# j-min/HiREST

Measured on AMD Instinct MI355X. Metric: encoded frames/sec (EVA-CLIP-g/14 224^2), higher is better.
Workload: dtype bf16

## Files before the change

### hirest_amd/_lib.py

```python
from __future__ import annotations

import ctypes as C
import os

HERE = os.path.dirname(os.path.abspath(__file__))
LIB_PATH = os.path.join(HERE, "lib", "libhirest_hip.so")
if os.environ.get("HIREST_LIB_VARIANT"):
    LIB_PATH = os.path.join(HERE, "lib", f"libhirest_hip.{os.environ['HIREST_LIB_VARIANT']}.so")

(EPI_BIAS_BF16, EPI_BIAS_GELU_BF16, EPI_BIAS_QGELU_BF16, EPI_BIAS_RESID_F32, EPI_BIAS_F32, EPI_PATCH_POS_F32,
 EPI_BIAS_RESID_LNSTATS_F32, EPI_LNFOLD_BF16, EPI_LNFOLD_GELU_BF16, EPI_BIAS_GELU_SPLIT2, EPI_BIAS_RESID2_LNSTATS) = range(11)

TOWER_NO_LNFOLD = 1
TOWER_NO_PRUNE = 2
TOWER_F32_RESIDUAL = 4
GEMM_REVERSE = 1
GEMM_X3 = 2
GEMM_X3_T128 = 4
ABI_VERSION = 4

ERRORS = {-1: "HIREST_E_BADARG", -2: "HIREST_E_SHAPE (unsupported shape)", -3: "HIREST_E_WORKSPACE (workspace too small)"}


class GemmArgs(C.Structure):
    _fields_ = [("struct_size", C.c_uint64),
                ("A", C.c_void_p), ("lda", C.c_int64), ("W", C.c_void_p), ("ldw", C.c_int64),
                ("bias", C.c_void_p), ("out", C.c_void_p), ("ldo", C.c_int64),
                ("M", C.c_int32), ("N", C.c_int32), ("K", C.c_int32), ("epilogue", C.c_int32),
                ("pos", C.c_void_p), ("patches_per_frame", C.c_int32), ("aux0", C.c_void_p), ("aux1", C.c_void_p), ("flags", C.c_int32)]

    @classmethod
    def make(cls, *fields):
        return cls(C.sizeof(cls), *fields)


F32_ENTRY = {"gemm": 0, "ws": 1, "layouts": 2, "ln": 3, "ln_colmax": 4, "rows_colmax": 5}


class GemmF32Query(C.Structure):
    _fields_ = [("struct_size", C.c_uint32)] + \
               [(n, C.c_int32) for n in ("entry", "M", "N", "K", "has_resid", "has_periodic", "has_ids", "has_ln_out", "has_workspace",
                                         "a_kmajor", "w_kmajor", "select_kernel", "ring_mode", "rows_ln_mode", "cus")]

    @classmethod
    def make(cls, entry, M, N, K, **fields):
        q = cls(C.sizeof(cls), F32_ENTRY[entry], M, N, K, select_kernel=-1, ring_mode=-1, rows_ln_mode=-1)
        for k, v in fields.items():
            setattr(q, k, int(v))
        return q


class BlockWeights(C.Structure):
    _fields_ = [(n, C.c_void_p) for n in ("ln1_g", "ln1_b", "qkv_w", "qkv_b", "proj_w", "proj_b",
                                          "ln2_g", "ln2_b", "fc1_w", "fc1_b", "fc2_w", "fc2_b",
                                          "qkv_wf", "qkv_bf", "qkv_s", "fc1_wf", "fc1_bf", "fc1_s")]


class VisionTower(C.Structure):
    _fields_ = [(n, C.c_int32) for n in ("image_size", "patch", "width", "heads", "head_dim", "mlp_dim",
                                         "layers", "embed_dim", "kpad", "act")] + \
               [("ln_eps", C.c_float)] + \
               [("patch_w", C.c_void_p), ("patch_b", C.c_void_p), ("cls", C.c_void_p), ("pos", C.c_void_p),
                ("blocks", C.POINTER(BlockWeights)),
                ("norm_g", C.c_void_p), ("norm_b", C.c_void_p), ("head_w", C.c_void_p), ("head_b", C.c_void_p),
                ("image_mean", C.c_void_p), ("image_std", C.c_void_p),
                ("ln_pre_g", C.c_void_p), ("ln_pre_b", C.c_void_p), ("out_all_tokens", C.c_int32)]


class TextTower(C.Structure):
    _fields_ = [(n, C.c_int32) for n in ("context", "vocab", "width", "heads", "layers", "embed_dim", "act")] + \
               [("ln_eps", C.c_float)] + \
# ... 495 lines not shown
```

### hirest_amd/csrc/gemm.hip

```cpp
#include <cstdio>
#include <atomic>
#include "gemm_shared.h"

namespace {


constexpr int BM = 128, BN = 128, BK = 64;
constexpr int STAGE_BYTES = (BM + BN) * BK * 2;

template <int EPI>
__device__ __forceinline__ void epilogue_store(const GemmP& p, int m, int n, f32x4 v) {
    if (p.bias) {
        f32x4 b = *reinterpret_cast<const f32x4*>(p.bias + n);
        v += b;
    }
    if constexpr (EPI == HIREST_EPI_BIAS_BF16 || EPI == HIREST_EPI_BIAS_GELU_BF16 || EPI == HIREST_EPI_BIAS_QGELU_BF16) {
        if constexpr (EPI == HIREST_EPI_BIAS_GELU_BF16) {
#pragma unroll
            for (int i = 0; i < 4; ++i) v[i] = gelu_erf(v[i]);
        }
        if constexpr (EPI == HIREST_EPI_BIAS_QGELU_BF16) {
#pragma unroll
            for (int i = 0; i < 4; ++i) v[i] = quick_gelu(v[i]);
        }
// ... 927 lines not shown
            if constexpr (epi_is_lnfold(EPI)) {
                int r0 = M0 + wr * 128 + 2 * lane;
                const int last = (p.M - 1) & ~1;
                r0 = r0 < last ? r0 : last;
                glds16(reinterpret_cast<const float*>(p.aux0) + 2 * (int64_t)r0, stg + P_STG);
            }
#pragma unroll
            for (int i = 0; i < 8; ++i)
#pragma unroll
                for (int jn = 0; jn < NI; ++jn) acc[i][jn] = f32x4{0.f, 0.f, 0.f, 0.f};
            load_frags(smem + (g & 1) * Q_STEP, 0, f0);
            for (int t = 0; t < nst; ++t, ++g) {
                const char* cur = smem + (g & 1) * Q_STEP;
                const char* nxt = smem + ((g + 1) & 1) * Q_STEP;
                __builtin_amdgcn_sched_barrier(0);
                if (!(dbg & 256)) load_frags(cur, 1, f1);
                mfma_half(f0);
#pragma unroll
                for (int i = 0; i < NR; ++i) {
                    __builtin_amdgcn_sched_group_barrier(0x008, 2, 0);
                    __builtin_amdgcn_sched_group_barrier(0x100, 1, 0);
                }
                __builtin_amdgcn_sched_barrier(0);
                if (!(dbg & 64)) HX_WAIT_VM(0);
                HX_WAIT_LGKM0();
                __builtin_amdgcn_s_barrier();
                __builtin_amdgcn_sched_barrier(0);
                stage();
                load_frags(nxt, 0, f0);
                mfma_half(f1);
                __builtin_amdgcn_sched_group_barrier(0x020, 2 * PPW, 0);
#pragma unroll
                for (int i = 0; i < NR; ++i) {
                    __builtin_amdgcn_sched_group_barrier(0x008, 1, 0);
                    __builtin_amdgcn_sched_group_barrier(0x100, 1, 0);
                }
                __builtin_amdgcn_sched_barrier(0);
                advance();
            }
            epilogue_p<EPI, NI, epi_is_lnfold(EPI), 8, RD, false, DBG>(p, acc, stg, M0 + wr * 128, N0 + wc * WN, lane);
        } else {
            for (int t = 0; t < nst; ++t, ++g) {
                HX_WAIT_VM(0);
                __builtin_amdgcn_s_barrier();
                stage();
                advance();
            }
        }
    }
    HX_WAIT_VM(0);
}


template <int EPI, int RD, bool X3, int PH2 = 0, bool DBG = false>
__device__ __forceinline__ void pp256_body(const GemmP& p) {
    constexpr int NI = 4;
    const int sched = DBG ? p.sched : 0, stagger = DBG ? p.stagger : 0;
    extern __shared__ __attribute__((aligned(16))) char smem[];
    const int tid = threadIdx.x, lane = tid & 63;
    const int wave = __builtin_amdgcn_readfirstlane(tid >> 6);
    const int grp = wave >> 2;
    const int wr = grp, wc = wave & 3;

    const int bid = blockIdx.x;
    const int xcd = bid & 7, slot = bid >> 3, nslot = gridDim.x >> 3;
    int p_lo, np;
    xcd_panels<DBG>(p, xcd, p_lo, np);
    if (np <= 0) return;
    const bool panel_major = p.nbn <= 8;
    const int nunit = np * p.nbn;
    if (slot >= nunit) return;
    const bool team_walk = DBG && (sched & 4) && panel_major && p.nbn <= nslot && nunit >= nslot;
    const int teams = team_walk ? nslot / p.nbn : 0, tslots = teams * p.nbn, solo = nslot - tslots;
    const int np_solo = team_walk && solo ? (np * solo + nslot / 2) / nslot : 0, np_team = np - np_solo;
    int count;
    if (!team_walk) count = (nunit - slot + nslot - 1) / nslot;
    else if (slot < tslots) { const int tm = slot / p.nbn; count = tm < np_team ? (np_team - tm + teams - 1) / teams : 0; }
    else { const int sl_ = slot - tslots; count = sl_ < np_solo ? ((np_solo - sl_ + solo - 1) / solo) * p.nbn : 0; }
    if (count <= 0) return;
    if (stagger) {
        const int who = stagger == 1 ? (slot & 3) : stagger == 2 ? (xcd & 3) : ((slot + xcd) & 7);
        const int units = who * (stagger == 3 ? (p.K / Q_BK + 15) / 16 : (p.K / Q_BK + 7) / 8);
        for (int i = 0; i < units; ++i) __builtin_amdgcn_s_sleep(127);
    }
    auto team_origin = [&](int i, int& M0, int& N0) {
        if (p.rev) i = count - 1 - i;
        int panel, col;
        if (slot < tslots) { panel = slot / p.nbn + i * teams; col = slot % p.nbn; }
        else { panel = np_team + (slot - tslots) + (i / p.nbn) * solo; col = i % p.nbn; }
        M0 = (p_lo + panel) * T_BM; N0 = col * T_BN;
    };
    auto tile_origin = [&](int j, int& M0, int& N0) {
        if (team_walk) { team_origin((j - slot) / nslot, M0, N0); return; }
        if (p.rev) j = nunit - 1 - j;
        if (panel_major) {
            const int mt_i = j / p.nbn;
            M0 = (p_lo + mt_i) * T_BM; N0 = (j - mt_i * p.nbn) * T_BN;
            return;
        }
        const int g_ = j / (GROUP_M * p.nbn);
        const int r = j - g_ * GROUP_M * p.nbn;
        int gcount = np - g_ * GROUP_M; gcount = gcount > GROUP_M ? GROUP_M : gcount;
        const int nt_i = r / gcount, mt_i = p_lo + g_ * GROUP_M + (r - nt_i * gcount);
        M0 = mt_i * T_BM; N0 = nt_i * T_BN;
    };

    const int nst = p.K / Q_BK;
    uint32_t a_off[2][2], w_off[2][2];
    int a_lds[2][2], w_lds[2][2];
    const char* a_base; const char* w_base;
#pragma unroll
    for (int hsel = 0; hsel < 2; ++hsel)
#pragma unroll
        for (int q = 0; q < 2; ++q) {
            const int j = 2 * wave + q;
            a_lds[hsel][q] = ((j >> 3) * 128 + hsel * 64 + (j & 7) * 8) * 128;
            w_lds[hsel][q] = Q_WOFF + ((j >> 2) * 64 + hsel * 32 + (j & 3) * 8) * 128;
        }
    auto set_sources = [&](int M0, int N0) {
#pragma unroll
        for (int hsel = 0; hsel < 2; ++hsel)
#pragma unroll
            for (int q = 0; q < 2; ++q) {
                const int ra0 = (a_lds[hsel][q] >> 7) + (lane >> 3);
                const int rw0 = ((w_lds[hsel][q] - Q_WOFF) >> 7) + (lane >> 3);
                const int ca = (lane & 7) ^ ((ra0 >> 1) & 7), cw = (lane & 7) ^ ((rw0 >> 1) & 7);
                int ra = p.M - 1 - M0; ra = ra0 < ra ? ra0 : ra;
                int rn = p.N - 1 - N0; rn = rw0 < rn ? rw0 : rn;
                a_off[hsel][q] = (uint32_t)(ra * (int)p.lda + ca * 8) * 2u;
                w_off[hsel][q] = (uint32_t)(rn * (int)p.ldw + cw * 8) * 2u;
            }
        const int Ma = (DBG && (sched & 8)) ? (p_lo + ((M0 / T_BM - p_lo) & 3)) * T_BM : M0;
// ... 28 lines not shown
            dma_j += nslot;
            if (dma_j < slot + count * nslot) { int m0, n0; tile_origin(dma_j, m0, n0); set_sources(m0, n0); dma_k = 0; }
            else { dma_live = false; dma_k = nst - 1; }
        }
    };

    const int frow = lane & 15, fsw = (frow >> 1) & 7, kg = lane >> 4;
    const int a_frag = (wr * 128 + frow) * (Q_BK * 2);
    const int w_frag = Q_WOFF + (wc * 64 + frow) * (Q_BK * 2);
    int koff[2];
#pragma unroll
    for (int h = 0; h < 2; ++h) koff[h] = ((4 * h + kg) ^ fsw) << 4;
    struct FA { bf16x8 v[4][2]; };
    struct FW { bf16x8 v[2][2]; };
    FA Af;
    FW W0, W1;
    auto read_a = [&](const char* buf, int a) {
#pragma unroll
        for (int m = 0; m < 4; ++m)
#pragma unroll
            for (int h = 0; h < 2; ++h) Af.v[m][h] = *reinterpret_cast<const bf16x8*>(buf + a_frag + (a * 64 + m * 16) * 128 + koff[h]);
    };
    auto read_w = [&](const char* buf, int b, FW& f) {
#pragma unroll
        for (int n = 0; n < 2; ++n)
#pragma unroll
            for (int h = 0; h < 2; ++h) f.v[n][h] = *reinterpret_cast<const bf16x8*>(buf + w_frag + (b * 32 + n * 16) * 128 + koff[h]);
    };
    f32x4 acc[8][NI];
    auto mfma_q = [&](int a, int b, FW& fw) {
        __builtin_amdgcn_s_setprio(1);
        if constexpr (X3) {
#pragma unroll
            for (int g3 = 0; g3 < 3; ++g3)
#pragma unroll
                for (int m = 0; m < 4; ++m)
#pragma unroll
                    for (int n = 0; n < 2; ++n)
                        acc[a * 4 + m][b * 2 + n] = __builtin_amdgcn_mfma_f32_16x16x32_bf16(fw.v[n][g3 == 1 ? 1 : 0], Af.v[m][g3 == 0 ? 1 : 0],
                                                                                             acc[a * 4 + m][b * 2 + n], 0, 0, 0);
        } else {
#pragma unroll
            for (int h = 0; h < 2; ++h)
#pragma unroll
                for (int m = 0; m < 4; ++m)
#pragma unroll
                    for (int n = 0; n < 2; ++n)
                        acc[a * 4 + m][b * 2 + n] = __builtin_amdgcn_mfma_f32_16x16x32_bf16(fw.v[n][h], Af.v[m][h], acc[a * 4 + m][b * 2 + n], 0, 0, 0);
        }
        __builtin_amdgcn_s_setprio(0);
    };
    auto bar = [&]() { __builtin_amdgcn_s_barrier(); };

    {
        int m0, n0;
        tile_origin(slot, m0, n0);
        set_sources(m0, n0);
    }
    for (int i = 0; i < 2; ++i) { issue_a0(); issue_w(0); issue_w(1); advance(); issue_a1_pending(); }
    bool a1_valid = false;
    HX_WAIT_VM(0);
    bar();
    if (grp == 1) bar();

    char* stg = smem + 2 * Q_STEP + wave * p_stg_bytes(EPI);
    int g = 0;
    for (int j = slot; j < slot + count * nslot; j += nslot) {
        int M0, N0;
        tile_origin(j, M0, N0);
        const bool active = (N0 + wc * 64 < p.N) && (M0 + wr * 128 < p.M);
        if (active) {
            if constexpr (epi_is_lnfold(EPI)) {
                int r0 = M0 + wr * 128 + 2 * lane;
                const int last = (p.M - 1) & ~1;
                r0 = r0 < last ? r0 : last;
                glds16(reinterpret_cast<const float*>(p.aux0) + 2 * (int64_t)r0, stg + P_STG);
                int c = N0 + wc * 64 + 4 * (lane & 15);
                c = c < p.N - 4 ? c : p.N - 4;
                const float* src = ((lane & 16) || !p.bias) ? reinterpret_cast<const float*>(p.aux1) : p.bias;
                glds16(src + c, stg + P_BCS);
            }
#pragma unroll
            for (int i = 0; i < 8; ++i)
#pragma unroll
                for (int jn = 0; jn < NI; ++jn) acc[i][jn] = f32x4{0.f, 0.f, 0.f, 0.f};
        }
        if (active && PH2) {
            for (int t = 0; t < nst; ++t, ++g) {
                const char* cur = smem + (g & 1) * Q_STEP;
                HX_WAIT_VM(6);
                __builtin_amdgcn_sched_barrier(0);
                read_a(cur, 0); read_w(cur, 0, W0); read_w(cur, 1, W1);
                if (a1_valid) issue_a1_pending();
                HX_WAIT_LGKM0();
                bar();
                mfma_q(0, 0, W0);
                mfma_q(0, 1, W1);
                bar();
                HX_WAIT_VM(2);
                __builtin_amdgcn_sched_barrier(0);
                read_a(cur, 1);
                issue_a0(); issue_w(0); issue_w(1);
                advance();
                a1_valid = true;
                HX_WAIT_LGKM0();
                bar();
// ... 18 lines not shown
                const char* cur = smem + (g & 1) * Q_STEP;
                HX_WAIT_VM(8);
                __builtin_amdgcn_sched_barrier(0);
                read_a(cur, 0); read_w(cur, 0, W0);
                if (a1_valid) issue_a1_pending();
                bar();
                HX_WAIT_LGKM0();
                mfma_q(0, 0, W0);
                bar();
                HX_WAIT_VM(8);
                __builtin_amdgcn_sched_barrier(0);
                read_w(cur, 1, W1);
                bar();
                HX_WAIT_LGKM0();
                mfma_q(0, 1, W1);
                bar();
                __builtin_amdgcn_sched_barrier(0);
                read_a(cur, 1);
                issue_a0(); issue_w(0);
                bar();
                HX_WAIT_LGKM0();
                mfma_q(1, 1, W1);
                bar();
                HX_WAIT_VM(8);
                __builtin_amdgcn_sched_barrier(0);
                issue_w(1);
                advance();
                a1_valid = true;
                bar();
                mfma_q(1, 0, W0);
                bar();
            }
            if constexpr (epi_is_lnfold(EPI)) HX_WAIT_VM(8);
            epilogue_p<EPI, NI, epi_is_lnfold(EPI), 8, RD, false, DBG, epi_is_lnfold(EPI)>(p, acc, stg, M0 + wr * 128, N0 + wc * 64, lane);
        } else {
            for (int t = 0; t < nst; ++t, ++g) {
                HX_WAIT_VM(8);
                if (a1_valid) issue_a1_pending();
                bar(); bar();
                HX_WAIT_VM(8);
                bar(); bar();
                issue_a0(); issue_w(0);
                bar(); bar();
                HX_WAIT_VM(8);
                issue_w(1);
                advance();
                a1_valid = true;
                bar(); bar();
            }
        }
    }
    if (grp == 0) bar();
    HX_WAIT_VM(0);
}

template <int EPI, int RD = 1>
__global__ __launch_bounds__(512) void gemm_pp256(GemmP p) { pp256_body<EPI, RD, false>(p); }
template <int EPI>
__global__ __launch_bounds__(512) void gemm_pp256x3(GemmP p) { pp256_body<EPI, 1, true>(p); }
template <int EPI>
__global__ __launch_bounds__(512) void gemm_pq256(GemmP p) { pp256_body<EPI, (EPI == HIREST_EPI_BIAS_RESID2_LNSTATS ? HIREST_S2_RD : 1), false, 1>(p); }
template <int EPI>
__global__ __launch_bounds__(512) void gemm_pq256x3(GemmP p) { pp256_body<EPI, 1, true, 1>(p); }
template <int EPI>
__global__ __launch_bounds__(512) void gemm_pq256_dbg(GemmP p) { pp256_body<EPI, (EPI == HIREST_EPI_BIAS_RESID2_LNSTATS ? HIREST_S2_RD : 1), false, 1, true>(p); }



static inline void tiles256(GemmP& p) {
    p.nbm = (p.M + T_BM - 1) / T_BM; p.nbn = (p.N + T_BN - 1) / T_BN;
    p.ppx = (p.nbm + 7) / 8;
}

template <auto KERN, int LDS>
int launch_tiles(GemmP p, hipStream_t s) {
    static HirestDevCfg cfg;
    if (int e = hirest_configure(KERN, LDS, cfg)) return e;
    tiles256(p);
    hipLaunchKernelGGL(KERN, dim3(8 * p.ppx * p.nbn), dim3(512), LDS, s, p);
    return hirest_launch_status();
}
template <auto KERN, int NW, int LDS>
int launch_persistent(GemmP p, hipStream_t s) {
    static HirestDevCfg cfg;
    int cus = 0;
    if (int e = hirest_configure(KERN, LDS, cfg, &cus)) return e;
    tiles256(p);
    int nslot = cus / 8; nslot = nslot < 1 ? 1 : nslot;
    const int per_xcd = p.ppx * p.nbn;
    if (nslot > per_xcd) nslot = per_xcd;
    hipLaunchKernelGGL(KERN, dim3(8 * nslot), dim3(64 * NW), LDS, s, p);
    return hirest_launch_status();
}
constexpr int p_lds(int epi, int nw) { return 2 * Q_STEP + nw * p_stg_bytes(epi); }

template <int EPI>
int launch_t128(GemmP p, hipStream_t s) {
    hipLaunchKernelGGL(gemm_t128<EPI>, dim3(8 * p.ppx * p.nbn), dim3(256), 2 * STAGE_BYTES, s, p);
    return hirest_launch_status();
}

template <int EPI, int WM>
int launch_t128x3(GemmP p, hipStream_t s) {
    static HirestDevCfg cfg;
    auto kern = gemm_t128x3<EPI, WM>;
    constexpr int LDS = 4 * (64 * WM + BN) * BK * 2;
    if (int e = hirest_configure(kern, LDS, cfg)) return e;
    p.nbm = (p.M + 64 * WM - 1) / (64 * WM);
    p.ppx = (p.nbm + 7) / 8;
    p.flat = p.nbm < 32 ? 1 : 0;
    p.ksplit = 1;
    if (EPI == HIREST_EPI_BIAS_RESID_F32 && p.flat && p.aux0 && !p.aux1) {
        const int ntile = p.nbm * p.nbn, nk = p.K / BK;
        for (int S = 4; S >= 2; --S)
            if (nk % S == 0 && nk / S >= 8 && ntile * S <= 256) { p.ksplit = S; break; }
        p.part = reinterpret_cast<float*>(p.aux0);
    }
    const int grid = p.flat ? 8 * ((p.nbm * p.nbn * p.ksplit + 7) / 8) : 8 * p.ppx * p.nbn;
    hipLaunchKernelGGL(kern, dim3(grid), dim3(256 * WM), LDS, s, p);
    if (p.ksplit > 1) {
        const int64_t total = (int64_t)p.M * (p.N / 4);
        int blocks = (int)((total + 255) / 256); blocks = blocks > 2048 ? 2048 : blocks;
        hipLaunchKernelGGL(splitk_reduce_kernel, dim3(blocks), dim3(256), 0, s, p.part, p.ksplit, p.bias, reinterpret_cast<float*>(p.out), p.ldo, p.M, p.N);
    }
    return hirest_launch_status();
}

}
std::atomic<int> g_force_kernel{0};
std::atomic<int> g_gemm_dbg{0};
namespace {

constexpr bool epi_is_plain(int e) { return e >= HIREST_EPI_BIAS_BF16 && e <= HIREST_EPI_PATCH_POS_F32; }
constexpr bool epi_is_fused(int e) { return e == HIREST_EPI_BIAS_RESID_LNSTATS_F32 || e == HIREST_EPI_BIAS_RESID2_LNSTATS || epi_is_lnfold(e); }
constexpr bool epi_is_x3(int e) { return e == HIREST_EPI_BIAS_F32 || e == HIREST_EPI_BIAS_RESID_F32 || e == HIREST_EPI_BIAS_GELU_SPLIT2; }
constexpr bool epi_has_p256_dbg(int e) { return e == HIREST_EPI_BIAS_BF16 || e == HIREST_EPI_BIAS_GELU_BF16 || e == HIREST_EPI_BIAS_RESID_F32; }

enum class GemmFamily { t128, t256, t256p, t256q, p256, pp256, pq256, pq256_dbg, pp256x3, pq256x3, t128x3 };
struct GemmChoice {
    int status = 0;
    GemmFamily family = GemmFamily::t128;
    int epi = 0;
    int ring = 0;
// ... 86 lines not shown
        default: break;
    }
    return {nullptr, nullptr};
}
GemmKernel gemm_kernel(const GemmChoice& c) {
    switch (c.epi) {
        case HIREST_EPI_BIAS_BF16: return gemm_kernel<HIREST_EPI_BIAS_BF16>(c);
        case HIREST_EPI_BIAS_GELU_BF16: return gemm_kernel<HIREST_EPI_BIAS_GELU_BF16>(c);
        case HIREST_EPI_BIAS_QGELU_BF16: return gemm_kernel<HIREST_EPI_BIAS_QGELU_BF16>(c);
        case HIREST_EPI_BIAS_RESID_F32: return gemm_kernel<HIREST_EPI_BIAS_RESID_F32>(c);
        case HIREST_EPI_BIAS_F32: return gemm_kernel<HIREST_EPI_BIAS_F32>(c);
        case HIREST_EPI_PATCH_POS_F32: return gemm_kernel<HIREST_EPI_PATCH_POS_F32>(c);
        case HIREST_EPI_BIAS_RESID_LNSTATS_F32: return gemm_kernel<HIREST_EPI_BIAS_RESID_LNSTATS_F32>(c);
        case HIREST_EPI_LNFOLD_BF16: return gemm_kernel<HIREST_EPI_LNFOLD_BF16>(c);
        case HIREST_EPI_LNFOLD_GELU_BF16: return gemm_kernel<HIREST_EPI_LNFOLD_GELU_BF16>(c);
        case HIREST_EPI_BIAS_GELU_SPLIT2: return gemm_kernel<HIREST_EPI_BIAS_GELU_SPLIT2>(c);
        case HIREST_EPI_BIAS_RESID2_LNSTATS: return gemm_kernel<HIREST_EPI_BIAS_RESID2_LNSTATS>(c);
        default: return {nullptr, nullptr};
    }
}

int epilogue_operand_status(const hirest_gemm_args& a) {
    const int e = a.epilogue;
    if (e == HIREST_EPI_PATCH_POS_F32 && (!a.pos || a.patches_per_frame <= 0)) return HIREST_E_BADARG;
    if (e == HIREST_EPI_BIAS_GELU_SPLIT2 && (a.N % 32 != 0 || a.ldo < 2 * (int64_t)a.N || a.ldo % 8 != 0)) return HIREST_E_SHAPE;
    if (epi_is_fused(e) && (!a.aux0 || !a.aux1)) return HIREST_E_BADARG;
    if ((e == HIREST_EPI_BIAS_RESID_LNSTATS_F32 || e == HIREST_EPI_BIAS_RESID2_LNSTATS) && a.N % 8 != 0) return HIREST_E_SHAPE;
    if (e == HIREST_EPI_BIAS_RESID2_LNSTATS && a.ldo % 8 != 0) return HIREST_E_SHAPE;
    if (epi_is_lnfold(e) && HIREST_LNFOLD_BUFFER_EPILOGUE && a.ldo >= ((int64_t)1 << 22)) return HIREST_E_SHAPE;
    return 0;
}

}

extern "C" int hirest_gemm_debug_mode(int32_t bits) { g_gemm_dbg = bits; return 0; }

extern "C" int hirest_gemm_select_kernel(int32_t which) {
    if (which < 0 || which > 9) return HIREST_E_BADARG;
    g_force_kernel = which;
    return 0;
}

extern "C" int hirest_gemm_dispatch_name(const hirest_gemm_args* a, char* out, int32_t out_len) {
    if (!a || a->struct_size != sizeof(hirest_gemm_args) || !out || out_len < 48) return HIREST_E_BADARG;
    const GemmChoice c = gemm_choose(*a);
    if (c.status) return c.status;
    snprintf(out, out_len, gemm_kernel(c).name, c.epi);
    return 0;
}

extern "C" int hirest_gemm_bf16(const hirest_gemm_args* a, void* stream) {
    if (!a || a->struct_size != sizeof(hirest_gemm_args) || !a->A || !a->W || !a->out) return HIREST_E_BADARG;
    if (a->M <= 0 || a->N <= 0 || a->K <= 0) return HIREST_E_BADARG;
    if (a->flags & ~(HIREST_GEMM_REVERSE | HIREST_GEMM_X3 | HIREST_GEMM_X3_T128)) return HIREST_E_BADARG;
    if ((a->flags & HIREST_GEMM_X3_T128) && !(a->flags & HIREST_GEMM_X3)) return HIREST_E_BADARG;
    if (a->K % BK != 0 || a->K % T_BK != 0 || a->N % 4 != 0 || a->lda % 8 != 0 || a->ldw % 8 != 0) return HIREST_E_SHAPE;
    if (a->ldo % 4 != 0) return HIREST_E_SHAPE;
    const GemmChoice c = gemm_choose(*a);
    const int word = g_gemm_dbg;
    GemmP p;
    p.A = reinterpret_cast<const bf16_t*>(a->A); p.lda = a->lda;
    p.W = reinterpret_cast<const bf16_t*>(a->W); p.ldw = a->ldw;
    p.bias = a->bias; p.out = a->out; p.ldo = a->ldo;
    p.M = a->M; p.N = a->N; p.K = a->K;
    p.pos = a->pos; p.P = a->patches_per_frame;
    p.aux0 = a->aux0; p.aux1 = a->aux1;
    p.rev = ((a->flags & HIREST_GEMM_REVERSE) && !(word & GEMM_DBG_IGNORE_REVERSE)) ? 1 : 0;
    p.dbg = c.drop_dbg ? 0 : word & GEMM_DBG_KERNEL_BITS;
    p.stagger = (word >> GEMM_DBG_STAGGER_SHIFT) & GEMM_DBG_STAGGER_MASK;
    p.epi_dbg = (word >> GEMM_DBG_EPI_SHIFT) & GEMM_DBG_EPI_MASK;
    p.sched = (word >> GEMM_DBG_SCHED_SHIFT) & GEMM_DBG_SCHED_MASK;
    p.nbm = (a->M + BM - 1) / BM; p.nbn = (a->N + BN - 1) / BN;
    p.ppx = (p.nbm + 7) / 8;
    hipStream_t s = reinterpret_cast<hipStream_t>(stream);
    HirestProfScope prof(HIREST_PROF_GEMM, a->epilogue, a->M, a->N, a->K, s);
    if (c.status) return c.status;
    if (int e = epilogue_operand_status(*a)) return e;
    return gemm_kernel(c).launch(p, s);
}
```

### hirest_amd/csrc/gemm_shared.h

```cpp
#pragma once
#include "common.h"
#include "profile.h"

namespace {

struct GemmP {
    const bf16_t* A; int64_t lda;
    const bf16_t* W; int64_t ldw;
    const float* bias;
    void* out; int64_t ldo;
    int M, N, K;
    const float* pos; int P;
    int rev;
    void* aux0; void* aux1;
    int nbm, nbn, ppx;
    int epi_dbg;
    int stagger;
    int sched;
    int dbg;
    int flat = 0;
    int ksplit = 1;
    float* part = nullptr;
};
constexpr int GEMM_DBG_IGNORE_REVERSE = 1 << 9;
constexpr int GEMM_DBG_STAGGER_SHIFT = 10, GEMM_DBG_STAGGER_MASK = 3;
constexpr int GEMM_DBG_EPI_SHIFT = 12, GEMM_DBG_EPI_MASK = 15;
constexpr int GEMM_DBG_SCHED_SHIFT = 16, GEMM_DBG_SCHED_MASK = 15;
constexpr int GEMM_DBG_PQ_SWITCHES = GEMM_DBG_STAGGER_MASK << GEMM_DBG_STAGGER_SHIFT | GEMM_DBG_EPI_MASK << GEMM_DBG_EPI_SHIFT | GEMM_DBG_SCHED_MASK << GEMM_DBG_SCHED_SHIFT;
constexpr int GEMM_DBG_KERNEL_BITS = ~(GEMM_DBG_IGNORE_REVERSE | GEMM_DBG_PQ_SWITCHES);

constexpr int GROUP_M = 8;
template <bool DBG = false>
__device__ __forceinline__ void xcd_panels(const GemmP& p, int xcd, int& p_lo, int& np) {
    if (DBG && (p.sched & 1)) { p_lo = xcd * p.ppx; np = p.nbm - p_lo; np = np > p.ppx ? p.ppx : np; return; }
    p_lo = (int)(((long long)xcd * p.nbm) >> 3);
    np = (int)(((long long)(xcd + 1) * p.nbm) >> 3) - p_lo;
}
constexpr int T_BM = 256, T_BN = 256;
#define HX_WAIT_VM(n) asm volatile("s_waitcnt vmcnt(" #n ")" ::: "memory")
#define HX_WAIT_LGKM0() asm volatile("s_waitcnt lgkmcnt(0)" ::: "memory")
constexpr int Q_BK = 64;
constexpr int Q_STEP = (T_BM + T_BN) * Q_BK * 2;
constexpr int Q_WOFF = T_BM * Q_BK * 2;

#ifndef HIREST_X3_GELU_POLY
#define HIREST_X3_GELU_POLY 1
#endif
#ifndef HIREST_S2_BUFFER_EPILOGUE
#define HIREST_S2_BUFFER_EPILOGUE 1
#endif
#ifndef HIREST_LNFOLD_BUFFER_EPILOGUE
#define HIREST_LNFOLD_BUFFER_EPILOGUE 1
#endif
#ifndef HIREST_S2_RD
#define HIREST_S2_RD 2
#endif
constexpr int P_STG = 2048;
constexpr bool epi_is_lnfold(int epi) { return epi == HIREST_EPI_LNFOLD_BF16 || epi == HIREST_EPI_LNFOLD_GELU_BF16; }
constexpr int P_BCS = P_STG + 1024;
constexpr int p_stg_bytes(int epi) {
    return epi_is_lnfold(epi) ? P_STG + 2048 : (epi == HIREST_EPI_BIAS_RESID2_LNSTATS && HIREST_S2_BUFFER_EPILOGUE) ? 2 * P_STG : P_STG;
}

#define HX_LDS_ORDER() asm volatile("" ::: "memory")

__device__ __forceinline__ float dpp_xor1(float v) {
    return __builtin_bit_cast(float, __builtin_amdgcn_mov_dpp(__builtin_bit_cast(int, v), 0xB1, 0xf, 0xf, true));
}
__device__ __forceinline__ float sum8(float v) {
    v += __builtin_bit_cast(float, __builtin_amdgcn_mov_dpp(__builtin_bit_cast(int, v), 0xB1, 0xf, 0xf, true));
    v += __builtin_bit_cast(float, __builtin_amdgcn_mov_dpp(__builtin_bit_cast(int, v), 0x4E, 0xf, 0xf, true));
    v += __builtin_bit_cast(float, __builtin_amdgcn_mov_dpp(__builtin_bit_cast(int, v), 0x141, 0xf, 0xf, true));
    return v;
}
typedef __attribute__((ext_vector_type(4))) unsigned u32x4;
typedef __attribute__((ext_vector_type(2))) unsigned u32x2;
constexpr unsigned HX_OOB = 0x80000000u;
__device__ __forceinline__ __amdgpu_buffer_rsrc_t hx_rsrc(const void* base, unsigned bytes) {
    return __builtin_amdgcn_make_buffer_rsrc(const_cast<void*>(base), 0, (int)bytes, 0x00020000);
}

template <int NI, int NM, int RD, bool S2 = false, bool DBG = false>
__device__ __forceinline__ void epilogue_lnstats(const GemmP& p, f32x4 (&acc)[8][NI], int jc, char* stg, int Mw, int Nw, int lane) {
    const int epi_dbg = DBG ? p.epi_dbg : 0, sched = DBG ? p.sched : 0;
    const int srow = lane & 15, kg = lane >> 4, sw = lane & 7;
    const int rr = lane >> 3, rc = lane & 7;
    float* outp = reinterpret_cast<float*>(p.out);
    bf16_t* xb = reinterpret_cast<bf16_t*>(p.aux0);
    float* part = reinterpret_cast<float*>(p.aux1);
    const int G = (p.N + 63) >> 6;
    f32x4 bv[4];
#pragma unroll
    for (int n = 0; n < 4; ++n) {
        const int col = Nw + n * 16 + 4 * kg;
        bv[n] = (p.bias && col < p.N) ? *reinterpret_cast<const f32x4*>(p.bias + col) : f32x4{0.f, 0.f, 0.f, 0.f};
    }
    const int n0 = Nw + rc * 4, n1 = Nw + 32 + rc * 4;
    bf16_t* xlo = reinterpret_cast<bf16_t*>(p.out);
    auto load_res = [&](int mi, f32x4 (&o)[2][2]) {
#pragma unroll
        for (int it = 0; it < 2; ++it) {
            const int m = Mw + mi * 16 + it * 8 + rr;
            if constexpr (S2) {
                const int64_t mr = m < p.M ? m : p.M - 1;
                const int col = (rc & 1) ? n1 - 4 : n0;
// ... 48 lines not shown
                *reinterpret_cast<f32x4*>(stg + srow * 128 + (((nn * 4 + kg) ^ sw) << 4)) = acc[mi][jc + h * 2 + nn] + bv[h * 2 + nn];
            HX_LDS_ORDER();
#pragma unroll
            for (int it = 0; it < 2; ++it) {
                const int r = it * 8 + rr;
                wv[h][it] = *reinterpret_cast<const f32x4*>(stg + r * 128 + ((rc ^ (r & 7)) << 4)) + oc[h][it];
            }
            HX_LDS_ORDER();
        }
#pragma unroll
        for (int it = 0; it < 2; ++it) {
            const int m = Mw + mi * 16 + it * 8 + rr;
            const bool okm = m < p.M, ok0 = okm && n0 < p.N, ok1 = okm && n1 < p.N;
            if constexpr (!S2) {
                if (ok0 && !(epi_dbg & 2)) __builtin_nontemporal_store(wv[0][it], reinterpret_cast<f32x4*>(outp + (int64_t)m * p.ldo + n0));
                if (ok1 && !(epi_dbg & 2)) __builtin_nontemporal_store(wv[1][it], reinterpret_cast<f32x4*>(outp + (int64_t)m * p.ldo + n1));
            }
            union { bf16x4 v; float f[2]; } b0, b1, snd, rcv;
            float ps = 0.f, pq = 0.f;
#pragma unroll
            for (int e = 0; e < 4; ++e) {
                b0.v[e] = (bf16_t)wv[0][it][e]; b1.v[e] = (bf16_t)wv[1][it][e];
                const float f0 = ok0 ? (float)b0.v[e] : 0.f, f1 = ok1 ? (float)b1.v[e] : 0.f;
                ps += f0 + f1; pq = fmaf(f0, f0, fmaf(f1, f1, pq));
            }
            snd.v = (rc & 1) ? b0.v : b1.v;
            rcv.f[0] = dpp_xor1(snd.f[0]); rcv.f[1] = dpp_xor1(snd.f[1]);
            union { bf16x8 v; float f[4]; } w8;
            int col;
            if (rc & 1) { w8.f[0] = rcv.f[0]; w8.f[1] = rcv.f[1]; w8.f[2] = b1.f[0]; w8.f[3] = b1.f[1]; col = n1 - 4; }
            else        { w8.f[0] = b0.f[0]; w8.f[1] = b0.f[1]; w8.f[2] = rcv.f[0]; w8.f[3] = rcv.f[1]; col = n0; }
            if (okm && col + 8 <= p.N && !(epi_dbg & 4)) __builtin_nontemporal_store(w8.v, reinterpret_cast<bf16x8*>(xb + (int64_t)m * p.N + col));
            if constexpr (S2) {
                union { bf16x4 v; float f[2]; } l0, l1, ls, lr;
#pragma unroll
                for (int e = 0; e < 4; ++e) {
                    l0.v[e] = (bf16_t)(wv[0][it][e] - (float)b0.v[e]);
                    l1.v[e] = (bf16_t)(wv[1][it][e] - (float)b1.v[e]);
                }
                ls.v = (rc & 1) ? l0.v : l1.v;
                lr.f[0] = dpp_xor1(ls.f[0]); lr.f[1] = dpp_xor1(ls.f[1]);
                union { bf16x8 v; float f[4]; } q8;
                if (rc & 1) { q8.f[0] = lr.f[0]; q8.f[1] = lr.f[1]; q8.f[2] = l1.f[0]; q8.f[3] = l1.f[1]; }
                else        { q8.f[0] = l0.f[0]; q8.f[1] = l0.f[1]; q8.f[2] = lr.f[0]; q8.f[3] = lr.f[1]; }
                if (okm && col + 8 <= p.N && !(epi_dbg & 2)) __builtin_nontemporal_store(q8.v, reinterpret_cast<bf16x8*>(xlo + (int64_t)m * p.ldo + col));
            }
            ps = sum8(ps); pq = sum8(pq);
            if (rc == 0 && okm && Nw < p.N && !(epi_dbg & 8)) *reinterpret_cast<f32x2*>(part + ((int64_t)m * G + (Nw >> 6)) * 2) = f32x2{ps, pq};
        }
    }
}


template <int NI, int NM, int RD, bool DBG = false>
__device__ __forceinline__ void epilogue_lnstats2(const GemmP& p, f32x4 (&acc)[8][NI], int jc, char* stg, int Mw, int Nw, int lane) {
    const int epi_dbg = DBG ? p.epi_dbg : 0, sched = DBG ? p.sched : 0;
    const int srow = lane & 15, kg = lane >> 4, sw = lane & 7;
    const int rr = lane >> 3, rc = lane & 7;
    const int G = (p.N + 63) >> 6;
    const int N = p.N, ldo = (int)p.ldo;
    int rows = p.M - Mw; rows = rows < NM * 16 ? rows : NM * 16;
    const __amdgpu_buffer_rsrc_t rs_hi = hx_rsrc(reinterpret_cast<const bf16_t*>(p.aux0) + (int64_t)Mw * N, (unsigned)rows * (unsigned)N * 2u);
    const __amdgpu_buffer_rsrc_t rs_lo = hx_rsrc(reinterpret_cast<const bf16_t*>(p.out) + (int64_t)Mw * ldo, ((unsigned)(rows - 1) * (unsigned)ldo + (unsigned)N) * 2u);
    const __amdgpu_buffer_rsrc_t rs_pt = hx_rsrc(reinterpret_cast<const float*>(p.aux1) + ((int64_t)Mw * G + (Nw >> 6)) * 2, ((unsigned)(rows - 1) * (unsigned)G + 1u) * 8u);
    const __amdgpu_buffer_rsrc_t rs_b = hx_rsrc(p.bias, p.bias ? (unsigned)N * 4u : 0u);
    const int n0 = Nw + rc * 4, n1 = Nw + 32 + rc * 4;
    const f32x4 bias0 = __builtin_bit_cast(f32x4, __builtin_amdgcn_raw_buffer_load_b128(rs_b, (unsigned)n0 * 4u, 0, 0));
    const f32x4 bias1 = __builtin_bit_cast(f32x4, __builtin_amdgcn_raw_buffer_load_b128(rs_b, (unsigned)n1 * 4u, 0, 0));
    const int col = (rc & 1) ? n1 - 4 : n0;
    const bool col_ok = col + 8 <= N;
    const unsigned vh0 = col_ok ? (unsigned)(rr * N + col) * 2u : HX_OOB, vl0 = col_ok ? (unsigned)(rr * ldo + col) * 2u : HX_OOB;
    const unsigned vp0 = (rc == 0 && Nw < N) ? (unsigned)(rr * G) * 8u : HX_OOB;
    const unsigned sh = 16u * (unsigned)N, sl = 16u * (unsigned)ldo, sp = 64u * (unsigned)G;
    const unsigned vh_ld = (epi_dbg & 1) ? HX_OOB : vh0, vl_ld = (epi_dbg & 1) ? HX_OOB : vl0;
    const unsigned vh_st = (epi_dbg & 4) ? HX_OOB : vh0, vl_st = (epi_dbg & 2) ? HX_OOB : vl0, vp_st = (epi_dbg & 8) ? HX_OOB : vp0;
    auto load_res = [&](int mi, u32x4 (&o)[2][2]) {
#pragma unroll
        for (int it = 0; it < 2; ++it) {
            const int k = mi * 2 + it;
            const bool okm = k * 8 + rr < rows;
            const unsigned vh = okm ? vh_ld : HX_OOB, vl = okm ? vl_ld : HX_OOB;
            if (DBG && (sched & 2)) {
                o[0][it] = __builtin_amdgcn_raw_buffer_load_b128(rs_hi, vh, (unsigned)k * sh, 0);
                o[1][it] = __builtin_amdgcn_raw_buffer_load_b128(rs_lo, vl, (unsigned)k * sl, 0);
            } else {
                o[0][it] = __builtin_amdgcn_raw_buffer_load_b128(rs_hi, vh, (unsigned)k * sh, 2);
                o[1][it] = __builtin_amdgcn_raw_buffer_load_b128(rs_lo, vl, (unsigned)k * sl, 2);
            }
        }
    };
    u32x4 ring[RD + 1][2][2];
#pragma unroll
    for (int a = 0; a < RD && a < NM; ++a) load_res(a, ring[a]);
#pragma unroll
    for (int mi = 0; mi < NM; ++mi) {
        if (mi + RD < NM) load_res(mi + RD, ring[(mi + RD) % (RD + 1)]);
        __builtin_amdgcn_sched_barrier(0);
#pragma unroll
        for (int h = 0; h < 2; ++h)
#pragma unroll
            for (int nn = 0; nn < 2; ++nn)
                *reinterpret_cast<f32x4*>(stg + h * P_STG + srow * 128 + (((nn * 4 + kg) ^ sw) << 4)) = acc[mi][jc + h * 2 + nn];
        HX_LDS_ORDER();
#pragma unroll
        for (int it = 0; it < 2; ++it) {
            const int k = mi * 2 + it;
            const int r = it * 8 + rr;
            f32x4 oc0, oc1;
// ... 281 lines not shown
            for (int n = 0; n < 2; ++n) {
                const int col = Nw + (jp + n) * 16 + 4 * kg;
                bv[n] = (p.bias && col < p.N) ? *reinterpret_cast<const f32x4*>(p.bias + col) : f32x4{0.f, 0.f, 0.f, 0.f};
            }
            const int n = Nw + jp * 16 + rc * 4;
#pragma unroll
            for (int mh = 0; mh < NM; mh += 4) {
                f32x4 o[8];
#pragma unroll
                for (int it = 0; it < 8; ++it) {
                    const int m = Mw + mh * 16 + it * 8 + rr;
                    const bool ok = m < p.M && n < p.N;
                    if constexpr (EPI == HIREST_EPI_PATCH_POS_F32) {
                        const int mm = ok ? m : 0;
                        const int pp = mm % p.P;
                        o[it] = ok ? *reinterpret_cast<const f32x4*>(p.pos + (int64_t)(1 + pp) * p.N + n) : f32x4{0.f, 0.f, 0.f, 0.f};
                    } else if constexpr (EPI == HIREST_EPI_BIAS_RESID_F32) {
                        o[it] = ok ? __builtin_nontemporal_load(reinterpret_cast<const f32x4*>(outp + (int64_t)m * p.ldo + n)) : f32x4{0.f, 0.f, 0.f, 0.f};
                    }
                }
#pragma unroll
                for (int mi = mh; mi < mh + 4; ++mi) {
#pragma unroll
                    for (int nn = 0; nn < 2; ++nn) {
                        const f32x4 v = acc[mi][jp + nn] + bv[nn];
                        *reinterpret_cast<f32x4*>(stg + srow * 128 + (((nn * 4 + kg) ^ sw) << 4)) = v;
                    }
                    HX_LDS_ORDER();
#pragma unroll
                    for (int it = 0; it < 2; ++it) {
                        const int r = it * 8 + rr;
                        f32x4 w = *reinterpret_cast<const f32x4*>(stg + r * 128 + ((rc ^ (r & 7)) << 4));
                        if constexpr (EPI != HIREST_EPI_BIAS_F32) w += o[(mi - mh) * 2 + it];
                        const int m = Mw + mi * 16 + r;
                        if (m < p.M && n < p.N) {
                            int64_t off;
                            if constexpr (EPI == HIREST_EPI_PATCH_POS_F32) {
                                const int b = m / p.P, pp = m - b * p.P;
                                off = ((int64_t)b * (p.P + 1) + 1 + pp) * p.ldo + n;
                            } else {
                                off = (int64_t)m * p.ldo + n;
                            }
                            __builtin_nontemporal_store(w, reinterpret_cast<f32x4*>(outp + off));
                        }
                    }
                    HX_LDS_ORDER();
                }
            }
        }
    }
}

}
```

### include/hirest_hip.h

```cpp
#ifndef HIREST_HIP_H
#define HIREST_HIP_H

#include <stddef.h>
#include <stdint.h>

#ifdef __cplusplus
extern "C" {
#endif

#define HIREST_ABI_VERSION 4

#define HIREST_E_BADARG   (-1)
#define HIREST_E_SHAPE    (-2)
#define HIREST_E_WORKSPACE (-3)

typedef uint16_t hirest_bf16;

int hirest_abi_version(void);
const char* hirest_build_info(void);

enum hirest_epilogue {
    HIREST_EPI_BIAS_BF16 = 0,
    HIREST_EPI_BIAS_GELU_BF16 = 1,
    HIREST_EPI_BIAS_QGELU_BF16 = 2,
    HIREST_EPI_BIAS_RESID_F32 = 3,
    HIREST_EPI_BIAS_F32 = 4,
    HIREST_EPI_PATCH_POS_F32 = 5,
    HIREST_EPI_BIAS_RESID_LNSTATS_F32 = 6,
    HIREST_EPI_LNFOLD_BF16 = 7,
    HIREST_EPI_LNFOLD_GELU_BF16 = 8,
    HIREST_EPI_BIAS_GELU_SPLIT2 = 9,
    HIREST_EPI_BIAS_RESID2_LNSTATS = 10
};

typedef struct hirest_gemm_args {
    uint64_t struct_size;
    const hirest_bf16* A;  int64_t lda;
    const hirest_bf16* W;  int64_t ldw;
    const float* bias;
    void* out;             int64_t ldo;
    int32_t M, N, K;
    int32_t epilogue;
    const float* pos;
    int32_t patches_per_frame;
    void* aux0;
    void* aux1;
    int32_t flags;
} hirest_gemm_args;
enum { HIREST_GEMM_REVERSE = 1,
       HIREST_GEMM_X3 = 2,
       HIREST_GEMM_X3_T128 = 4
     };

int hirest_gemm_bf16(const hirest_gemm_args* args, void* stream);
int hirest_gemm_select_kernel(int32_t which);
int hirest_gemm_debug_mode(int32_t bits);
int hirest_gemm_dispatch_name(const hirest_gemm_args* args, char* out, int32_t out_len);

int hirest_layernorm(const float* x, int64_t ldx, const int32_t* row_index,
                     const float* gamma, const float* beta, float eps,
                     void* out, int64_t ldo, int32_t out_is_f32,
                     int32_t rows, int32_t D, void* stream);

int hirest_attention_bf16(const hirest_bf16* qkv, hirest_bf16* out,
                          int32_t B, int32_t N, int32_t H, int32_t dh,
                          float scale, int32_t causal, void* stream);
int hirest_attention_bf16_rows(const hirest_bf16* qkv, hirest_bf16* out,
                               int32_t B, int32_t N, int32_t H, int32_t dh,
                               float scale, int32_t causal, int32_t q_rows, void* stream);
int hirest_attention_bf16_long(const hirest_bf16* qkv, hirest_bf16* out, int32_t B, int32_t N, int32_t H, int32_t dh,
                               float scale, int32_t q_rows, void* stream);
int hirest_attention_select_kernel(int32_t which);
int hirest_attention_set_mapping(int32_t by_head);
int hirest_attention_set_pace(int32_t units);
int hirest_attention_set_stagger(int32_t units);
int hirest_attention_set_skew(int32_t units);
int hirest_attention_debug_mode(int32_t bits);
int hirest_attention_debug_trace_read(int64_t* dst, int32_t n);

int hirest_patchify(const void* frames, int32_t in_dtype, int32_t B, int32_t S, int32_t P,
                    const float* mean3, const float* std3,
                    hirest_bf16* patches, int32_t Kpad, void* stream);

int hirest_fold_layernorm(const float* W, const float* gamma, const float* beta, const float* bias, hirest_bf16* Wf,
                          float* bias_out, float* colsum_out, int32_t N, int32_t K, void* stream);
int hirest_write_cls_rows(float* x, int64_t ldx, const float* cls, const float* pos0,
                          int32_t B, int32_t tokens_per_frame, int32_t D, void* stream);

int hirest_rowstats_bf16(const float* x, int64_t ldx, hirest_bf16* xb, float* stats, float eps, int32_t rows, int32_t D,
                         float* guard, void* stream);
int hirest_rowstats_split_bf16(const float* x, int64_t ldx, hirest_bf16* xb, hirest_bf16* xlo, float* stats, float eps, int32_t rows,
                               int32_t D, float* guard, void* stream);
int hirest_combine_hi_lo_f32(const hirest_bf16* hi, const hirest_bf16* lo, int64_t ld_in, float* out, int64_t ldo, int32_t rows,
                             int32_t D, void* stream);
int hirest_ln_stats_finalize(const float* partials, int32_t groups, float* stats, float eps, int32_t rows, int32_t D,
                             float* guard, void* stream);

int hirest_embed_tokens(const int64_t* tokens, const float* tok_emb, const float* pos,
                        float* x, int32_t* eot_row, int32_t B, int32_t L, int32_t D,
                        int32_t vocab, void* stream);

int hirest_f32_to_bf16(const float* in, hirest_bf16* out, int64_t n, void* stream);

int hirest_pool_l2norm(const float* frame_embeds, float* out, int32_t V, int32_t F, int32_t E,
// ... 679 lines not shown
```

Baseline: 2192.

## Split leftover GEMM tail tiles into quarter-width pieces across extra persistent slots

Result: no change. 2204, median of 6 (+0.5%).

```diff
diff --git a/hirest_amd/_lib.py b/hirest_amd/_lib.py
--- a/hirest_amd/_lib.py
+++ b/hirest_amd/_lib.py
@@ -17,6 +17,8 @@
 GEMM_REVERSE = 1
 GEMM_X3 = 2
 GEMM_X3_T128 = 4
+GEMM_NO_TAIL = 16
+GEMM_DBG_NO_TAIL = 1 << 20
 ABI_VERSION = 4
 
 ERRORS = {-1: "HIREST_E_BADARG", -2: "HIREST_E_SHAPE (unsupported shape)", -3: "HIREST_E_WORKSPACE (workspace too small)"}
diff --git a/hirest_amd/csrc/gemm.hip b/hirest_amd/csrc/gemm.hip
--- a/hirest_amd/csrc/gemm.hip
+++ b/hirest_amd/csrc/gemm.hip
@@ -1003,6 +1003,96 @@
 }
 
 
+constexpr int QT_STEP = (T_BM + HX_QCOLS) * Q_BK * 2;
+static_assert(3 * QT_STEP <= 2 * Q_STEP, "the tail pass's three slots live in the main loop's ring");
+template <int EPI, int RD>
+__device__ __forceinline__ void pq256_tail(const GemmP& p, char* smem) {
+    const int tid = threadIdx.x, lane = tid & 63;
+    const int wave = __builtin_amdgcn_readfirstlane(tid >> 6);
+    const int grp = wave >> 2, wc = wave & 3;
+    const int bid = blockIdx.x;
+    int M0, N0;
+    if (!hx_tail_quarter(p.nbm, p.nbn, p.N, gridDim.x >> 3, bid & 7, p.rev, bid >> 3, M0, N0)) return;
+    const int nst = p.K / Q_BK;
+    uint32_t a_off[2][2], w_off;
+    int a_lds[2][2];
+#pragma unroll
+    for (int hsel = 0; hsel < 2; ++hsel)
+#pragma unroll
+        for (int q = 0; q < 2; ++q) {
+            const int j = 2 * wave + q;
+            a_lds[hsel][q] = ((j >> 3) * 128 + hsel * 64 + (j & 7) * 8) * 128;
+            const int ra0 = (a_lds[hsel][q] >> 7) + (lane >> 3);
+            const int ca = (lane & 7) ^ ((ra0 >> 1) & 7);
+            int ra = p.M - 1 - M0; ra = ra0 < ra ? ra0 : ra;
+            a_off[hsel][q] = (uint32_t)(ra * (int)p.lda + ca * 8) * 2u;
+        }
+    const int w_lds = Q_WOFF + wave * 8 * 128;
+    {
+        const int rw0 = wave * 8 + (lane >> 3);
+        const int cw = (lane & 7) ^ ((rw0 >> 1) & 7);
+        int rn = p.N - 1 - N0; rn = rw0 < rn ? rw0 : rn;
+        w_off = (uint32_t)(rn * (int)p.ldw + cw * 8) * 2u;
+    }
+    const char* a_base = reinterpret_cast<const char*>(p.A + (int64_t)M0 * p.lda);
+    const char* w_base = reinterpret_cast<const char*>(p.W + (int64_t)N0 * p.ldw);
+    auto issue = [&](int k, int s) {
+        k = k < nst ? k : nst - 1;
+        char* buf = smem + s * QT_STEP;
+        const char* ab = a_base + (int64_t)k * (Q_BK * 2);
+        const char* wb = w_base + (int64_t)k * (Q_BK * 2);
+        glds16(ab + a_off[0][0], buf + a_lds[0][0]);
+        glds16(ab + a_off[0][1], buf + a_lds[0][1]);
+        glds16(ab + a_off[1][0], buf + a_lds[1][0]);
+        glds16(ab + a_off[1][1], buf + a_lds[1][1]);
+        glds16(wb + w_off, buf + w_lds);
+    };
+    const int frow = lane & 15, fsw = (frow >> 1) & 7, kg = lane >> 4;
+    const int a_frag = (grp * 128 + wc * 32 + frow) * (Q_BK * 2);
+    const int w_frag = Q_WOFF + frow * (Q_BK * 2);
+    int koff[2];
+#pragma unroll
+    for (int h = 0; h < 2; ++h) koff[h] = ((4 * h + kg) ^ fsw) << 4;
+    f32x4 acc[2][4];
+#pragma unroll
+    for (int m = 0; m < 2; ++m)
+#pragma unroll
+        for (int n = 0; n < 4; ++n) acc[m][n] = f32x4{0.f, 0.f, 0.f, 0.f};
+    issue(0, 0);
+    issue(1, 1);
+    int s = 0, s2 = 2;
+    for (int g = 0; g < nst; ++g) {
+        HX_WAIT_VM(5);
+        __builtin_amdgcn_s_barrier();
+        __builtin_amdgcn_sched_barrier(0);
+        issue(g + 2, s2);
+        const char* cur = smem + s * QT_STEP;
+        bf16x8 af[2][2], wf[4][2];
+#pragma unroll
+        for (int m = 0; m < 2; ++m)
+#pragma unroll
+            for (int h = 0; h < 2; ++h) af[m][h] = *reinterpret_cast<const bf16x8*>(cur + a_frag + m * 16 * 128 + koff[h]);
+#pragma unroll
+        for (int n = 0; n < 4; ++n)
+#pragma unroll
+            for (int h = 0; h < 2; ++h) wf[n][h] = *reinterpret_cast<const bf16x8*>(cur + w_frag + n * 16 * 128 + koff[h]);
+        HX_WAIT_LGKM0();
+        __builtin_amdgcn_sched_barrier(0);
+#pragma unroll
+        for (int h = 0; h < 2; ++h)
+#pragma unroll
+            for (int m = 0; m < 2; ++m)
+#pragma unroll
+                for (int n = 0; n < 4; ++n)
+                    acc[m][n] = __builtin_amdgcn_mfma_f32_16x16x32_bf16(wf[n][h], af[m][h], acc[m][n], 0, 0, 0);
+        s = s == 2 ? 0 : s + 1;
+        s2 = s2 == 2 ? 0 : s2 + 1;
+    }
+    const int Mw = M0 + grp * 128 + wc * 32;
+    if (Mw < p.M) epilogue_lnstats2<4, 2, RD>(p, acc, 0, smem + 2 * Q_STEP + wave * p_stg_bytes(EPI), Mw, N0, lane);
+    HX_WAIT_VM(0);
+}
+
 template <int EPI, int RD, bool X3, int PH2 = 0, bool DBG = false>
 __device__ __forceinline__ void pp256_body(const GemmP& p) {
     constexpr int NI = 4;
@@ -1017,18 +1107,21 @@
     const int xcd = bid & 7, slot = bid >> 3, nslot = gridDim.x >> 3;
     int p_lo, np;
     xcd_panels<DBG>(p, xcd, p_lo, np);
+    constexpr bool TAIL = EPI == HIREST_EPI_BIAS_RESID2_LNSTATS && HIREST_S2_BUFFER_EPILOGUE && PH2 && !X3 && !DBG;
     if (np <= 0) return;
     const bool panel_major = p.nbn <= 8;
     const int nunit = np * p.nbn;
-    if (slot >= nunit) return;
+    int u_tail = 0;
+    if constexpr (TAIL) { if (p.tail) u_tail = hx_tail_surplus(nunit, nslot); }
+    if (!u_tail && slot >= nunit) return;
     const bool team_walk = DBG && (sched & 4) && panel_major && p.nbn <= nslot && nunit >= nslot;
     const int teams = team_walk ? nslot / p.nbn : 0, tslots = teams * p.nbn, solo = nslot - tslots;
     const int np_solo = team_walk && solo ? (np * solo + nslot / 2) / nslot : 0, np_team = np - np_solo;
     int count;
-    if (!team_walk) count = (nunit - slot + nslot - 1) / nslot;
+    if (!team_walk) count = (nunit - u_tail - slot + nslot - 1) / nslot;
     else if (slot < tslots) { const int tm = slot / p.nbn; count = tm < np_team ? (np_team - tm + teams - 1) / teams : 0; }
     else { const int sl_ = slot - tslots; count = sl_ < np_solo ? ((np_solo - sl_ + solo - 1) / solo) * p.nbn : 0; }
-    if (count <= 0) return;
+    if (!u_tail && count <= 0) return;
     if (stagger) {
         const int who = stagger == 1 ? (slot & 3) : stagger == 2 ? (xcd & 3) : ((slot + xcd) & 7);
         const int units = who * (stagger == 3 ? (p.K / Q_BK + 15) / 16 : (p.K / Q_BK + 7) / 8);
@@ -1163,6 +1256,7 @@
     };
     auto bar = [&]() { __builtin_amdgcn_s_barrier(); };
 
+    if (!TAIL || count > 0) {
     {
         int m0, n0;
         tile_origin(slot, m0, n0);
@@ -1287,6 +1381,14 @@
     }
     if (grp == 0) bar();
     HX_WAIT_VM(0);
+    }
+    if constexpr (TAIL) {
+        if (u_tail) {
+            HX_WAIT_LGKM0();
+            bar();
+            pq256_tail<EPI, RD>(p, smem);
+        }
+    }
 }
 
 template <int EPI, int RD = 1>
@@ -1321,9 +1423,7 @@
     int cus = 0;
     if (int e = hirest_configure(KERN, LDS, cfg, &cus)) return e;
     tiles256(p);
-    int nslot = cus / 8; nslot = nslot < 1 ? 1 : nslot;
-    const int per_xcd = p.ppx * p.nbn;
-    if (nslot > per_xcd) nslot = per_xcd;
+    const int nslot = hx_persistent_nslot(cus / 8, p.ppx, p.nbn, p.tail);
     hipLaunchKernelGGL(KERN, dim3(8 * nslot), dim3(64 * NW), LDS, s, p);
     return hirest_launch_status();
 }
@@ -1516,7 +1616,7 @@
 extern "C" int hirest_gemm_bf16(const hirest_gemm_args* a, void* stream) {
     if (!a || a->struct_size != sizeof(hirest_gemm_args) || !a->A || !a->W || !a->out) return HIREST_E_BADARG;
     if (a->M <= 0 || a->N <= 0 || a->K <= 0) return HIREST_E_BADARG;
-    if (a->flags & ~(HIREST_GEMM_REVERSE | HIREST_GEMM_X3 | HIREST_GEMM_X3_T128)) return HIREST_E_BADARG;
+    if (a->flags & ~(HIREST_GEMM_REVERSE | HIREST_GEMM_X3 | HIREST_GEMM_X3_T128 | HIREST_GEMM_NO_TAIL)) return HIREST_E_BADARG;
     if ((a->flags & HIREST_GEMM_X3_T128) && !(a->flags & HIREST_GEMM_X3)) return HIREST_E_BADARG;
     if (a->K % BK != 0 || a->K % T_BK != 0 || a->N % 4 != 0 || a->lda % 8 != 0 || a->ldw % 8 != 0) return HIREST_E_SHAPE;
     if (a->ldo % 4 != 0) return HIREST_E_SHAPE;
@@ -1530,6 +1630,8 @@
     p.pos = a->pos; p.P = a->patches_per_frame;
     p.aux0 = a->aux0; p.aux1 = a->aux1;
     p.rev = ((a->flags & HIREST_GEMM_REVERSE) && !(word & GEMM_DBG_IGNORE_REVERSE)) ? 1 : 0;
+    p.tail = (HIREST_GEMM_TAIL && c.family == GemmFamily::pq256 && c.epi == HIREST_EPI_BIAS_RESID2_LNSTATS && HIREST_S2_BUFFER_EPILOGUE &&
+              !(a->flags & HIREST_GEMM_NO_TAIL) && !(word & GEMM_DBG_NO_TAIL)) ? 1 : 0;
     p.dbg = c.drop_dbg ? 0 : word & GEMM_DBG_KERNEL_BITS;
     p.stagger = (word >> GEMM_DBG_STAGGER_SHIFT) & GEMM_DBG_STAGGER_MASK;
     p.epi_dbg = (word >> GEMM_DBG_EPI_SHIFT) & GEMM_DBG_EPI_MASK;
diff --git a/hirest_amd/csrc/gemm_shared.h b/hirest_amd/csrc/gemm_shared.h
--- a/hirest_amd/csrc/gemm_shared.h
+++ b/hirest_amd/csrc/gemm_shared.h
@@ -1,4 +1,48 @@
 #pragma once
+
+#if defined(__HIPCC__)
+#define HX_HD __host__ __device__ inline __attribute__((always_inline))
+#else
+#define HX_HD inline
+#endif
+namespace {
+constexpr int HX_TILE = 256, HX_GROUP_M = 8, HX_QCOLS = 64;
+HX_HD void hx_xcd_split(int nbm, int xcd, int& p_lo, int& np) {
+    p_lo = (int)(((long long)xcd * nbm) >> 3);
+    np = (int)(((long long)(xcd + 1) * nbm) >> 3) - p_lo;
+}
+HX_HD void hx_unit_origin(int j, int np, int nbn, int rev, int& panel, int& col) {
+    if (rev) j = np * nbn - 1 - j;
+    if (nbn <= 8) { panel = j / nbn; col = j - panel * nbn; return; }
+    const int g_ = j / (HX_GROUP_M * nbn);
+    const int r = j - g_ * HX_GROUP_M * nbn;
+    int gcount = np - g_ * HX_GROUP_M; gcount = gcount > HX_GROUP_M ? HX_GROUP_M : gcount;
+    col = r / gcount; panel = g_ * HX_GROUP_M + (r - col * gcount);
+}
+HX_HD int hx_tail_surplus(int nunit, int nslot) {
+    const int u = nunit % nslot;
+    return (u > 0 && 4 * u <= nslot) ? u : 0;
+}
+HX_HD bool hx_tail_quarter(int nbm, int nbn, int N, int nslot, int xcd, int rev, int slot, int& M0, int& N0) {
+    int p_lo, np;
+    hx_xcd_split(nbm, xcd, p_lo, np);
+    const int nunit = np * nbn, u = hx_tail_surplus(nunit, nslot);
+    const int s = slot >> 2, c = slot & 3;
+    if (s >= u) return false;
+    int panel, col;
+    hx_unit_origin(nunit - u + s, np, nbn, rev, panel, col);
+    M0 = (p_lo + panel) * HX_TILE; N0 = col * HX_TILE + c * HX_QCOLS;
+    return N0 < N;
+}
+HX_HD int hx_persistent_nslot(int cu_slots, int ppx, int nbn, int tail) {
+    if (cu_slots < 1) cu_slots = 1;
+    const int per_xcd = ppx * nbn;
+    if (cu_slots <= per_xcd) return cu_slots;
+    return (tail && 4 * per_xcd <= cu_slots) ? 4 * per_xcd : per_xcd;
+}
+}
+
+#ifndef HIREST_GEMM_PLAN_ONLY
 #include "common.h"
 #include "profile.h"
 
@@ -21,22 +65,23 @@
     int flat = 0;
     int ksplit = 1;
     float* part = nullptr;
+    int tail = 0;
 };
 constexpr int GEMM_DBG_IGNORE_REVERSE = 1 << 9;
 constexpr int GEMM_DBG_STAGGER_SHIFT = 10, GEMM_DBG_STAGGER_MASK = 3;
 constexpr int GEMM_DBG_EPI_SHIFT = 12, GEMM_DBG_EPI_MASK = 15;
 constexpr int GEMM_DBG_SCHED_SHIFT = 16, GEMM_DBG_SCHED_MASK = 15;
+constexpr int GEMM_DBG_NO_TAIL = 1 << 20;
 constexpr int GEMM_DBG_PQ_SWITCHES = GEMM_DBG_STAGGER_MASK << GEMM_DBG_STAGGER_SHIFT | GEMM_DBG_EPI_MASK << GEMM_DBG_EPI_SHIFT | GEMM_DBG_SCHED_MASK << GEMM_DBG_SCHED_SHIFT;
-constexpr int GEMM_DBG_KERNEL_BITS = ~(GEMM_DBG_IGNORE_REVERSE | GEMM_DBG_PQ_SWITCHES);
-
-constexpr int GROUP_M = 8;
+constexpr int GEMM_DBG_KERNEL_BITS = ~(GEMM_DBG_IGNORE_REVERSE | GEMM_DBG_NO_TAIL | GEMM_DBG_PQ_SWITCHES);
+
+constexpr int GROUP_M = HX_GROUP_M;
 template <bool DBG = false>
 __device__ __forceinline__ void xcd_panels(const GemmP& p, int xcd, int& p_lo, int& np) {
     if (DBG && (p.sched & 1)) { p_lo = xcd * p.ppx; np = p.nbm - p_lo; np = np > p.ppx ? p.ppx : np; return; }
-    p_lo = (int)(((long long)xcd * p.nbm) >> 3);
-    np = (int)(((long long)(xcd + 1) * p.nbm) >> 3) - p_lo;
-}
-constexpr int T_BM = 256, T_BN = 256;
+    hx_xcd_split(p.nbm, xcd, p_lo, np);
+}
+constexpr int T_BM = HX_TILE, T_BN = HX_TILE;
 #define HX_WAIT_VM(n) asm volatile("s_waitcnt vmcnt(" #n ")" ::: "memory")
 #define HX_WAIT_LGKM0() asm volatile("s_waitcnt lgkmcnt(0)" ::: "memory")
 constexpr int Q_BK = 64;
@@ -51,6 +96,9 @@
 #endif
 #ifndef HIREST_LNFOLD_BUFFER_EPILOGUE
 #define HIREST_LNFOLD_BUFFER_EPILOGUE 1
+#endif
+#ifndef HIREST_GEMM_TAIL
+#define HIREST_GEMM_TAIL 1
 #endif
 #ifndef HIREST_S2_RD
 #define HIREST_S2_RD 2
@@ -205,8 +253,8 @@
 }
 
 
-template <int NI, int NM, int RD, bool DBG = false>
-__device__ __forceinline__ void epilogue_lnstats2(const GemmP& p, f32x4 (&acc)[8][NI], int jc, char* stg, int Mw, int Nw, int lane) {
+template <int NI, int NM, int RD, bool DBG = false, int NR = 8>
+__device__ __forceinline__ void epilogue_lnstats2(const GemmP& p, f32x4 (&acc)[NR][NI], int jc, char* stg, int Mw, int Nw, int lane) {
     const int epi_dbg = DBG ? p.epi_dbg : 0, sched = DBG ? p.sched : 0;
     const int srow = lane & 15, kg = lane >> 4, sw = lane & 7;
     const int rr = lane >> 3, rc = lane & 7;
@@ -594,3 +642,4 @@
 }
 
 }
+#endif
diff --git a/include/hirest_hip.h b/include/hirest_hip.h
--- a/include/hirest_hip.h
+++ b/include/hirest_hip.h
@@ -49,7 +49,8 @@
 } hirest_gemm_args;
 enum { HIREST_GEMM_REVERSE = 1,
        HIREST_GEMM_X3 = 2,
-       HIREST_GEMM_X3_T128 = 4
+       HIREST_GEMM_X3_T128 = 4,
+       HIREST_GEMM_NO_TAIL = 16
      };
 
 int hirest_gemm_bf16(const hirest_gemm_args* args, void* stream);
```
